# MRIRC/MRI-super-resolution

Measured on AMD Instinct MI355X. Metric: voxels/sec per INR fit (128^3, x4 upscale): train coordinate-steps/s, higher is better.
Workload: dtype f32 as 3 x f16 MFMA products (hi/lo split operands, f32 accumulate); 1 GPU; synthetic 128^3 volume, LR 64x64x128 (N=524288 coords) -> x4 grid 256x256x128; Siren(256,512,3,1) + 128 Fourier features, Adam 1e-4, full-batch MSE; per_gpu_rows=524288, parallelism=1 independent fits (one volume per GPU)

## Files before the change

### mri-super-resolution_amd/csrc/gemm_hp.hip

```cpp
#include "internal.h"
#include "split_fp16.h"

namespace inr {

#include "gemm_hp.inc"
#include "gemm_hp_nt.inc"
#include "gemm_hp_row.inc"
#include "gemm_hp_fwd.inc"

int hp_build_flags() {
    int f = 0;
    if (HP_ABLATE != 0) f |= 2;
    if (HP_A_AUX != 2 || HP_MUL_AUX != 0 || HP_RC_A_AUX != 0 || HP_RC_B_AUX != 0 || HP_HEAD_NT != 0 || HP_UNSCALE_LDEXP != 1 || HP_HEAD_PREFETCH != 1 || HP_COLSUM_TRANSPOSED != 1 || HP_DIAG_NO_OMEGA_STASH != 0) f |= 8;
    return f;
}
tune_int g_stamp_class{-1}, g_stamp_nth{0};
static unsigned long long* hp_stamp_target(int kernel_class) {
    if (!g_stamps || kernel_class != g_stamp_class) return nullptr;
    return g_stamp_nth-- == 0 ? g_stamps : nullptr;
}

tune_int g_hp_stagger{0};
tune_int g_hp_persistent{2};
static int hp_num_cus() {
    static int n = 0;
    if (!n) {
        int dev = 0;
        hipDeviceProp_t prop;
        if (hipGetDevice(&dev) == hipSuccess && hipGetDeviceProperties(&prop, dev) == hipSuccess) n = prop.multiProcessorCount;
        if (n <= 0) n = 256;
    }
    return n;
}
tune_int g_hp_grid_cap{0};
static unsigned hp_persistent_grid(long long tiles) {
    long long g = tiles < hp_num_cus() ? tiles : hp_num_cus();
    const int cap = g_hp_grid_cap;
    if (cap > 0 && g > cap) g = cap;
    return (unsigned)g;
}
bool hp_head_ok(int hidden) { return hidden == 128 || hidden == 256 || hidden == 512 || hidden == 1024; }

size_t hp_prep_part_bytes() { return (size_t)8 * HP_PREP_MAXB * 2 * sizeof(unsigned); }
int hp_weight_prep(const float* const* W, const int* out_f, const int* in_f, int layers, char* planes, HpSlots slots,
                   unsigned* part, float* head_bound, const float* head_W, const float* head_b, int hidden, const unsigned* tmax,
                   const unsigned* wtmax, float inv_count, float omega, hipStream_t stream, const float* const* bias,
// ... 89 lines not shown
    }
    return c;
}

static HpParams hp_kc_params(char* c_hl, const char* a_hl, const char* b_hl, int64_t rows, int width, int k, HpScale sa, HpScale sb,
                             HpScale so, int kernel_class) {
    HpParams p{};
    p.A = a_hl; p.B = b_hl; p.C_hl = c_hl;
    p.M = (int)rows; p.N = width; p.K = k;
    p.pitchA = (long long)k * 4; p.pitchB = (long long)k * 4;
    p.a_rows = rows; p.b_rows = width;
    p.sa = sa; p.sb = sb; p.so = so;
    p.k_per_split = k; p.splits = 1; p.stagger = g_hp_stagger;
    p.stamps = hp_stamp_target(kernel_class);
    return p;
}

template <int EPI>
static int hp_launch_kc(HpParams p, const HpKcChoice& c, hipStream_t stream) {
    constexpr bool INLINE_EPI = EPI == HPE_SINE || EPI == HPE_SINE_STASH || EPI == HPE_MUL;
    const bool narrow = c.family == LF_HP_NARROW;
    const int bm = narrow ? NT_BM : HP_BM, bn = narrow ? NT_BN : HP_BN;
    p.tiles_m = (int)((p.a_rows + bm - 1) / bm);
    p.tiles_n = c.family == LF_HP_ROW ? 1 : (p.N + bn - 1) / bn;
    if (narrow) p.fold_bias = c.fold_bias;
    if (int rc = hp_check_grid(p)) return rc;
    const long long tiles = (long long)p.tiles_m * p.tiles_n;
    const dim3 grid((unsigned)tiles), pgrid(hp_persistent_grid(tiles)), block(narrow ? NT_NTH : HP_NTH);
    bool served = false;
    if (c.family == LF_HP_ROW) {
        hipLaunchKernelGGL((gemm_hp_row_kernel<EPI>), pgrid, block, 0, stream, p);
        served = true;
    }
    if constexpr (EPI != HPE_HEAD) {
        if (c.family == LF_HP_PKD && c.kt == 16) {
            hipLaunchKernelGGL((gemm_hp_pkd_kernel<EPI, 16>), pgrid, block, 0, stream, p);
            served = true;
        } else if (c.family == LF_HP_NARROW) {
            if (c.xzy) hipLaunchKernelGGL((gemm_hp_nt_kernel<EPI, true>), grid, block, 0, stream, p);
            else hipLaunchKernelGGL((gemm_hp_nt_kernel<EPI, false>), grid, block, 0, stream, p);
            served = true;
        }
        if constexpr (EPI != HPE_MUL) {
            if (c.family == LF_HP_PKD && c.kt == 8) {
                hipLaunchKernelGGL((gemm_hp_pkd_kernel<EPI, 8>), pgrid, block, 0, stream, p);
                served = true;
            }
        }
    }
    if constexpr (INLINE_EPI) {
        if (c.family == LF_HP_PKC) {
            hipLaunchKernelGGL((gemm_hp_pkc_kernel<EPI>), pgrid, block, 0, stream, p);
            served = true;
        } else if (c.family == LF_HP_TILE) {
            hipLaunchKernelGGL((gemm_hp_kernel<HP_KC, EPI>), grid, block, 0, stream, p);
            served = true;
        }
    }
    INR_REQUIRE(served, INR_E_INVALID, "hp gemm: no kernel of family %d for epilogue %d at K = %d", c.family, EPI, p.K);
    INR_LAUNCH_CHECK();
    count_launch(c.family);
    return 0;
}

int hp_sine_forward(char* act_hl, float* dact, const char* x_hl, const char* W_hl, const float* bias, int64_t n, int in_f,
                    int out_f, float omega, HpScale sa, HpScale sb, int reverse_m, hipStream_t stream, bool z_only, HpScale so) {
// ... 291 lines not shown
```

### mri-super-resolution_amd/csrc/gemm_hp.inc

```
__device__ __forceinline__ int hp_f(int r) {
    const int p = (r >> 1) & 7;
    return (p & 1) ^ (((p >> 1) & 1) * 5) ^ (((p >> 2) & 1) * 7);
}
__device__ __forceinline__ int hp_f2(int r) { return (r & 3) | (((r >> 3) & 1) << 2); }

#ifndef HP_A_AUX
#define HP_A_AUX 2
#endif
#ifndef HP_HEAD_NT
#define HP_HEAD_NT 0
#endif
#ifndef HP_RC_A_AUX
#define HP_RC_A_AUX 0
#endif
#ifndef HP_RC_B_AUX
#define HP_RC_B_AUX 0
#endif
#ifndef HP_MUL_AUX
#define HP_MUL_AUX 0
#endif
#ifndef HP_COLSUM_TRANSPOSED
#define HP_COLSUM_TRANSPOSED 1
#endif
#ifndef HP_HEAD_PREFETCH
#define HP_HEAD_PREFETCH 1
#endif
#ifndef HP_UNSCALE_LDEXP
#define HP_UNSCALE_LDEXP 1
#endif
#ifndef HP_DIAG_NO_OMEGA_STASH
#define HP_DIAG_NO_OMEGA_STASH 0
#endif
#ifndef HP_ABLATE
#define HP_ABLATE 0
#endif
enum HpMode { HP_KC = 0, HP_RC = 1 };
enum HpEpi { HPE_SINE = 0, HPE_SINE_STASH = 1, HPE_MUL = 2, HPE_SLAB = 3, HPE_Z = 4, HPE_HEAD = 5 };

__device__ __forceinline__ int hp_scale_exp(const HpScale& s) {
    if (s.mul == 0.f) return 0;
    float b = s.mul;
    if (s.meas) b *= __uint_as_float(*s.meas);
    if (s.wn) b *= *s.wn;
    if (!s.wn) return h3_scale_exp(__float_as_uint(b));
    return h3_scale_exp(__float_as_uint(b), s.kmax, -126);
}

__device__ __forceinline__ void hp_atomic_max_bits(unsigned* slot, float v) {
    const unsigned b = __float_as_uint(v);
    if (b > __hip_atomic_load(slot, __ATOMIC_RELAXED, __HIP_MEMORY_SCOPE_AGENT)) atomicMax(slot, b);
}

struct HpParams {
    const char* A;
    const char* B;
    int M, N, K;
    long long pitchA, pitchB;
    long long a_rows, b_rows;
    HpScale sa, sb, so;
    char* C_hl;
    float* C2;
    const float* bias;
    const float* mul;
    float* colsum;
    unsigned* amax_out;
    float omega;
    int tiles_m, tiles_n, splits;
    int k_per_split;
// ... 37 lines not shown
template <int ROWB>
__device__ __forceinline__ half8 hp_tr_read2(const char* lds) {
    typedef unsigned int u32x2 __attribute__((ext_vector_type(2)));
    u32x2 a, b;
    const unsigned addr = (unsigned)(unsigned long long)(__attribute__((address_space(3))) const char*)lds;
    asm volatile("ds_read_b64_tr_b16 %0, %1" : "=v"(a) : "v"(addr));
    asm volatile("ds_read_b64_tr_b16 %0, %1 offset:%2" : "=v"(b) : "v"(addr), "n"(4 * ROWB));
    return __builtin_bit_cast(half8, u32x4{a[0], a[1], b[0], b[1]});
}


__device__ __forceinline__ f32x4 hp_mul_sum(const f32x4& a, const f32x4& b, f32x4& cs) {
#pragma clang fp contract(off)
    const f32x4 o = a * b;
    cs = cs + o;
    return o;
}

__device__ __forceinline__ void hp_split8(const float (&v)[8], float s, u32x4& hi, u32x4& lo) {
    half2v h[4], l[4];
#pragma unroll
    for (int e = 0; e < 4; ++e) h3_split2<true>(v[2 * e], v[2 * e + 1], s, h[e], l[e]);
    hi = __builtin_bit_cast(u32x4, h);
    lo = __builtin_bit_cast(u32x4, l);
}
__device__ __forceinline__ void hp_split8_unit(const float (&v)[8], u32x4& hi, u32x4& lo) {
    half2v h[4], l[4];
#pragma unroll
    for (int e = 0; e < 4; ++e) h3_split2<false>(v[2 * e], v[2 * e + 1], 1.f, h[e], l[e]);
    hi = __builtin_bit_cast(u32x4, h);
    lo = __builtin_bit_cast(u32x4, l);
}

template <int MODE, int EPI>
__device__ __forceinline__ void gemm_hp_body(const HpParams& p, const int block_x) {
    constexpr int EPI_BYTES = 8 * 64 * SUB16 * 4;
    constexpr int SMEM_BYTES = HP_NSTAGE * HP_STAGE > EPI_BYTES ? HP_NSTAGE * HP_STAGE : EPI_BYTES;
    __shared__ __attribute__((aligned(1024))) char smem[SMEM_BYTES];
    constexpr bool KC = MODE == HP_KC;
    constexpr int A_ROWB = KC ? 128 : 512, B_ROWB = KC ? 128 : 1024;

    const int tid = threadIdx.x;
    const int lane = tid & 63, wave = __builtin_amdgcn_readfirstlane(tid >> 6);
    const int wm = wave >> 2, wn = wave & 3;
    const int g = lane >> 4, l16 = lane & 15;

    const int total = p.tiles_m * p.tiles_n * p.splits;
    int logical = xcd_remap(block_x, total);
    int tile_n = logical % p.tiles_n;
    logical /= p.tiles_n;
    int tile_m = logical % p.tiles_m;
    int split = logical / p.tiles_m;
    if (p.reverse_m) {
        if (p.splits > 1) split = p.splits - 1 - split;
        else tile_m = p.tiles_m - 1 - tile_m;
    }
    const int m0 = tile_m * HP_BM, n0 = tile_n * HP_BN;
    const int k_begin = split * p.k_per_split;
    const int k_end = min(p.K, k_begin + p.k_per_split);
    const int ktiles = (k_end - k_begin + HP_BK - 1) / HP_BK;

    __amdgpu_buffer_rsrc_t srdA, srdB;
    int step_a, step_b;
    if (KC) {
        srdA = hp_srd(p.A + (long long)m0 * p.pitchA, (p.a_rows - m0) * p.pitchA);
        srdB = hp_srd(p.B + (long long)n0 * p.pitchB, (p.b_rows - n0) * p.pitchB);
        step_a = step_b = 128;
    } else {
        const long long ra = min((long long)(k_end - k_begin), p.a_rows - k_begin);
        srdA = hp_srd(p.A + (long long)k_begin * p.pitchA + (m0 >> 5) * 128, ra * p.pitchA - (m0 >> 5) * 128);
        srdB = hp_srd(p.B + (long long)k_begin * p.pitchB + (n0 >> 5) * 128, ra * p.pitchB - (n0 >> 5) * 128);
        step_a = (int)(32 * p.pitchA);
        step_b = (int)(32 * p.pitchB);
    }
    int vdma[6];
#pragma unroll
    for (int i = 0; i < 6; ++i) {
        const int q = wave + 8 * i;
        if (KC) {
            const int row = 8 * (i < 2 ? q : q - 16) + (lane >> 3);
            const int c = (lane & 7) ^ hp_f(row);
            vdma[i] = row * (int)(i < 2 ? p.pitchA : p.pitchB) + c * 16;
        } else if (i < 2) {
            const int row = 2 * q + (lane >> 5), u = lane & 31;
            const int ch = (u >> 1) ^ hp_f2(row);
            vdma[i] = row * (int)p.pitchA + ch * 32 + (u & 1) * 16;
        } else {
            const int row = q - 16, u = lane;
            const int ch = (u >> 1) ^ hp_f2(row);
            vdma[i] = row * (int)p.pitchB + ch * 32 + (u & 1) * 16;
        }
    }
    int soff_a = KC ? (k_begin >> 5) * 128 : 0, soff_b = soff_a;
    auto dma_part = [&](int stage, int part) {
        char* S = smem + stage * HP_STAGE;
#pragma unroll
        for (int i = 0; i < 6; ++i) {
            if ((i >> 1) != part) continue;
            const int q = wave + 8 * i;
            if (!KC && i < 2)
                __builtin_amdgcn_raw_ptr_buffer_load_lds(srdA, (__attribute__((address_space(3))) void*)(S + q * 1024), 16, vdma[i],
                                                         soff_a, 0, HP_RC_A_AUX);
            else if (!KC)
                __builtin_amdgcn_raw_ptr_buffer_load_lds(srdB, (__attribute__((address_space(3))) void*)(S + q * 1024), 16, vdma[i],
                                                         soff_b, 0, HP_RC_B_AUX);
            else
                __builtin_amdgcn_raw_ptr_buffer_load_lds(i < 2 ? srdA : srdB, (__attribute__((address_space(3))) void*)(S + q * 1024),
                                                         16, vdma[i], i < 2 ? soff_a : soff_b, 0, 0);
        }
        if (part == 2) {
            soff_a += step_a;
            soff_b += step_b;
        }
    };
    auto dma = [&](int stage) {
        dma_part(stage, 0);
        dma_part(stage, 1);
        dma_part(stage, 2);
    };

    int fa[KC ? 2 : 8], fb[KC ? 2 : 8];
    if (KC) {
        const int fx = (g ^ hp_f(l16)) << 4;
        fa[0] = (64 * wm + l16) * 128 + fx;
        fa[1] = fa[0] ^ 64;
        fb[0] = HP_A_IMG + (64 * wn + l16) * 128 + fx;
        fb[1] = fb[0] ^ 64;
    } else {
        const int q = l16 >> 2, p4 = l16 & 3, row = 8 * g + q, f2 = hp_f2(row);
#pragma unroll
        for (int t = 0; t < 4; ++t)
#pragma unroll
            for (int lo = 0; lo < 2; ++lo) {
                const int mi = 4 * wm + t, ca = 4 * (mi >> 1) + (mi & 1) + 2 * lo;
                fa[2 * t + lo] = row * 512 + (ca ^ f2) * 32 + p4 * 8;
                const int ni = 4 * wn + t, cb = 4 * (ni >> 1) + (ni & 1) + 2 * lo;
                fb[2 * t + lo] = HP_A_IMG + row * 1024 + (cb ^ f2) * 32 + p4 * 8;
            }
    }
    auto frag_a = [&](const char* S, int i, int lo) -> half8 {
        if (KC) return *reinterpret_cast<const half8*>(S + fa[lo] + i * 2048);
        return hp_tr_read2<512>(S + fa[2 * i + lo]);
    };
    auto frag_b = [&](const char* S, int i, int lo) -> half8 {
        if (KC) return *reinterpret_cast<const half8*>(S + fb[lo] + i * 2048);
        return hp_tr_read2<1024>(S + fb[2 * i + lo]);
// ... 6 lines not shown
        for (int j = 0; j < 4; ++j) acc[i][j] = f32x4v{0.f, 0.f, 0.f, 0.f};
    half8 ah[2][4], bh[2][4], al[4], bl[4];

    HP_STAMP(0);
    if (ktiles > 0) dma(0);
    if (ktiles > 1) dma(1);
    if (ktiles > 2) dma(2);
    if (ktiles > 2) __builtin_amdgcn_s_waitcnt(0x0F70 | 12);
    else if (ktiles > 1) __builtin_amdgcn_s_waitcnt(0x0F70 | 6);
    else __builtin_amdgcn_s_waitcnt(0x0F70);
    __builtin_amdgcn_s_barrier();
    if (ktiles > 0) {
#pragma unroll
        for (int i = 0; i < 4; ++i) {
            ah[0][i] = frag_a(smem, i, 0);
            bl[i] = frag_b(smem, i, 1);
            al[i] = frag_a(smem, i, 1);
            bh[0][i] = frag_b(smem, i, 0);
        }
    }
    HP_STAMP(1);

    constexpr int NRD = KC ? 8 : 16;
    auto body = [&](auto par_c, auto st_c, int t) {
        constexpr int PAR = decltype(par_c)::value, ST = decltype(st_c)::value;
        const char* S1 = smem + ((ST + 1) % 3) * HP_STAGE;
        const bool more3 = t + 3 < ktiles;
        if (t == 7) HP_STAMP(5);
        if (t + 2 < ktiles) __builtin_amdgcn_s_waitcnt(0x0070 | 6);
        else __builtin_amdgcn_s_waitcnt(0x0070);
        __builtin_amdgcn_s_barrier();
        __builtin_amdgcn_sched_barrier(0);
        if (t == 7) HP_STAMP(6);
        if (more3) dma_part(ST, 0);
        h3_mfma16(acc, ah[PAR], bl);
        __builtin_amdgcn_sched_barrier(0);
        if (t == 7) HP_STAMP(7);
        if (more3) dma_part(ST, 1);
        if (KC) {
#pragma unroll
            for (int i = 0; i < 4; ++i) {
                bl[i] = frag_b(S1, i, 1);
                ah[PAR ^ 1][i] = frag_a(S1, i, 0);
            }
            h3_mfma16(acc, al, bh[PAR]);
            h3_sched<16, 0, 0, NRD, 0, 0>();
        } else {
#pragma unroll
            for (int i = 0; i < 4; ++i)
#pragma unroll
                for (int j = 0; j < 4; ++j) {
                    acc[i][j] = __builtin_amdgcn_mfma_f32_16x16x32_f16(al[i], bh[PAR][j], acc[i][j], 0, 0, 0);
                    if (j == 1) bl[i] = frag_b(S1, i, 1);
                    if (j == 3) ah[PAR ^ 1][i] = frag_a(S1, i, 0);
                }
        }
        __builtin_amdgcn_sched_barrier(0);
        if (t == 7) HP_STAMP(8);
        if (more3) dma_part(ST, 2);
        if (KC) {
#pragma unroll
            for (int i = 0; i < 4; ++i) {
                al[i] = frag_a(S1, i, 1);
                bh[PAR ^ 1][i] = frag_b(S1, i, 0);
            }
            h3_mfma16(acc, ah[PAR], bh[PAR]);
            h3_sched<16, 0, 0, NRD, 0, 0>();
        } else {
#pragma unroll
            for (int i = 0; i < 4; ++i)
#pragma unroll
                for (int j = 0; j < 4; ++j) {
                    acc[i][j] = __builtin_amdgcn_mfma_f32_16x16x32_f16(ah[PAR][i], bh[PAR][j], acc[i][j], 0, 0, 0);
                    if (j == 1) al[i] = frag_a(S1, i, 1);
                    if (j == 3) bh[PAR ^ 1][i] = frag_b(S1, i, 0);
                }
        }
        __builtin_amdgcn_sched_barrier(0);
        if (t == 7) HP_STAMP(9);
    };
    {
        using I0 = std::integral_constant<int, 0>;
        using I1 = std::integral_constant<int, 1>;
        using I2 = std::integral_constant<int, 2>;
        int t = 0;
        for (; t + 6 <= ktiles; t += 6) {
            body(I0{}, I0{}, t);
            body(I1{}, I1{}, t + 1);
            body(I0{}, I2{}, t + 2);
            body(I1{}, I0{}, t + 3);
            body(I0{}, I1{}, t + 4);
            body(I1{}, I2{}, t + 5);
        }
        if (t < ktiles) {
            body(I0{}, I0{}, t);
            if (t + 1 < ktiles) {
                body(I1{}, I1{}, t + 1);
                if (t + 2 < ktiles) {
                    body(I0{}, I2{}, t + 2);
                    if (t + 3 < ktiles) {
// ... 848 lines not shown
    while (true) {
        int t = 0;
        for (; t + 1 < ktiles; t += 2) {
            body(P0{}, t);
            body(P1{}, t + 1);
        }
        if (t < ktiles) {
            body(P0{}, t);
#pragma unroll
            for (int i = 0; i < 4; ++i) {
                ah[0][i] = ah[1][i];
                bh[0][i] = bh[1][i];
            }
        }
        HP_STAMP(2);
        if (!(HP_ABLATE & 4)) epilogue();
        else if (acc[0][0][0] == 12345.678f) p.C_hl[0] = (char)acc[1][1][1];
        HP_STAMP(4);
        if (!has_next) break;
        if (nxt.n0 != cur.n0) load_bias(nxt.n0);
        zero_acc();
        pend = 1;
        cur = nxt;
        vp += G;
        has_next = vp + G < total;
        if (has_next) nxt = decode(vp + G);
    }
    if (EPI == HPE_MUL && p.amax_out) {
        omax_run = wave_max(omax_run);
        if (lane == 0) hp_atomic_max_bits(p.amax_out, omax_run);
    }
}

template <int I, int N, typename F>
__device__ __forceinline__ void hp_static_for(F&& f) {
    if constexpr (I < N) {
        f(std::integral_constant<int, I>{});
        hp_static_for<I + 1, N>(f);
    }
}

template <int EPI, int KT>
__global__ void __launch_bounds__(HP_NTH, 2) gemm_hp_pkd_kernel(const HpParams p) {
    __shared__ __attribute__((aligned(1024))) char smem[HP_NSTAGE * HP_STAGE + 8 * HP_EPI_WAVE];
    constexpr int STORES = EPI == HPE_SINE_STASH ? 4 : 2;
    static_assert(EPI != HPE_SLAB, "row-split slabs are the one-block-per-tile kernel's business");
    constexpr int MULS = EPI == HPE_MUL ? 2 : 0;

    const int tid = threadIdx.x;
    const int lane = tid & 63, wave = __builtin_amdgcn_readfirstlane(tid >> 6);
    const int wm = wave >> 2, wn = wave & 3;
    const int g = lane >> 4, l16 = lane & 15;
    const int total = p.tiles_m * p.tiles_n;
    const int G = gridDim.x;

    struct Tile {
        int m0, n0;
        __amdgpu_buffer_rsrc_t srdA, srdB;
    };
    auto decode = [&](int vp) {
        int logical = xcd_remap(vp, total);
        Tile t;
        const int tn = logical % p.tiles_n, tm = logical / p.tiles_n;
        t.m0 = (p.reverse_m ? p.tiles_m - 1 - tm : tm) * HP_BM;
        t.n0 = tn * HP_BN;
        t.srdA = hp_srd(p.A + (long long)t.m0 * p.pitchA, (p.a_rows - t.m0) * p.pitchA);
        t.srdB = hp_srd(p.B + (long long)t.n0 * p.pitchB, (p.b_rows - t.n0) * p.pitchB);
        return t;
    };
    int vp = blockIdx.x;
    Tile cur = decode(vp), nxt = cur;
    bool has_next = vp + G < total;
    if (has_next) nxt = decode(vp + G);
    int prv_m0 = 0, prv_n0 = 0;
    bool have_prev = false;

    const int drow = 8 * wave + (lane >> 3);
    const int dslot = ((lane & 7) ^ hp_f(drow)) * 16;
    const int vdmaA = drow * (int)p.pitchA + dslot, vdmaB = drow * (int)p.pitchB + dslot;
    const int pieceA = 64 * (int)p.pitchA, pieceB = 64 * (int)p.pitchB;
    auto dma_part = [&](int stage_off, int j, int part) {
        char* S = smem + stage_off;
        const bool from_next = j >= KT;
        const int soff = (from_next ? j - KT : j) * 128;
        const __amdgpu_buffer_rsrc_t sa = from_next ? nxt.srdA : cur.srdA, sb = from_next ? nxt.srdB : cur.srdB;
#pragma unroll
        for (int i = 0; i < 6; ++i) {
            if ((i >> 1) != part) continue;
            const int q = wave + 8 * i;
            if (i < 2)
                __builtin_amdgcn_raw_ptr_buffer_load_lds(sa, (__attribute__((address_space(3))) void*)(S + q * 1024), 16, vdmaA,
                                                         soff + i * pieceA, 0, HP_A_AUX);
            else
                __builtin_amdgcn_raw_ptr_buffer_load_lds(sb, (__attribute__((address_space(3))) void*)(S + q * 1024), 16, vdmaB,
                                                         soff + (i - 2) * pieceB, 0, 0);
        }
    };

    const int fx = (g ^ hp_f(l16)) << 4;
    const int fa_hi = (64 * wm + l16) * 128 + fx, fa_lo = fa_hi ^ 64;
    const int fb_hi = HP_A_IMG + (64 * wn + l16) * 128 + fx, fb_lo = fb_hi ^ 64;

    const int ka = hp_scale_exp(p.sa), kb = hp_scale_exp(p.sb);
    float bias_s[4] = {0.f, 0.f, 0.f, 0.f};
    auto load_bias = [&](int n0) {
        if (EPI == HPE_MUL || !p.bias) return;
        const float upa = h3_pow2(ka), upb = h3_pow2(kb);
#pragma unroll
        for (int j = 0; j < 4; ++j) {
            const int col = n0 + 64 * wn + 16 * j + l16;
            const float b = p.bias[col < p.N ? col : p.N - 1];
            bias_s[j] = col < p.N ? (b * upa) * upb : 0.f;
        }
    };
    load_bias(cur.n0);
    f32x4v acc[4][4], accP[4][4];
    half8 ah[4], al[4], bh[4], bl[4];
    auto init_acc = [&]() {
#pragma unroll
        for (int i = 0; i < 4; ++i)
#pragma unroll
            for (int j = 0; j < 4; ++j) acc[i][j] = f32x4v{bias_s[j], bias_s[j], bias_s[j], bias_s[j]};
    };
    init_acc();

    const int er = lane >> 2, ec = (lane & 3) * 8;
    float* const stg = reinterpret_cast<float*>(smem + HP_NSTAGE * HP_STAGE + wave * HP_EPI_WAVE);
    const float inv_a = h3_pow2(-ka), inv_b = h3_pow2(-kb);
    const float so = h3_pow2(hp_scale_exp(p.so));
    f32x4 mul0 = {0.f, 0.f, 0.f, 0.f}, mul1 = mul0;
    f32x4 cs0 = {0.f, 0.f, 0.f, 0.f}, cs1 = cs0;
    float omax_run = 0.f;

    auto load_mul = [&](int c, f32x4& d0, f32x4& d1) {
        const __amdgpu_buffer_rsrc_t srdMul =
            hp_srd((const char*)p.mul + (long long)prv_m0 * p.N * 4, (long long)min(p.M - prv_m0, HP_BM) * p.N * 4);
        const int row = 64 * wm + 16 * (c & 3) + er, cc = prv_n0 + 64 * wn + 32 * (c >> 2) + ec;
        const int vo = cc < p.N ? (row * p.N + cc) * 4 : 0x7FFFFF00;
        d0 = __builtin_bit_cast(f32x4, __builtin_amdgcn_raw_buffer_load_b128(srdMul, vo, 0, HP_MUL_AUX));
        d1 = __builtin_bit_cast(f32x4, __builtin_amdgcn_raw_buffer_load_b128(srdMul, vo + 16, 0, HP_MUL_AUX));
    };
    auto chunk_park = [&](auto cc) {
        constexpr int c = decltype(cc)::value, i = c & 3, jp = c >> 2;
#pragma unroll
        for (int jj = 0; jj < 2; ++jj)
#pragma unroll
            for (int r = 0; r < 4; ++r)
                stg[(4 * g + r) * 32 + jj * 16 + l16] =
                    HP_UNSCALE_LDEXP ? __builtin_amdgcn_ldexpf(accP[i][2 * jp + jj][r], -(ka + kb)) : accP[i][2 * jp + jj][r] * inv_a * inv_b;
    };
    f32x4 cv0, cv1;
    auto chunk_read = [&]() {
        __builtin_amdgcn_s_waitcnt(0xC07F);
        __builtin_amdgcn_wave_barrier();
        cv0 = *reinterpret_cast<const f32x4*>(stg + er * 32 + ec);
        cv1 = *reinterpret_cast<const f32x4*>(stg + er * 32 + ec + 4);
    };
    auto chunk_finish = [&](auto cc) {
        constexpr int c = decltype(cc)::value, i = c & 3, jp = c >> 2;
        const long long first = (long long)prv_m0 * p.N * 4;
        const long long win = (long long)min(p.M - prv_m0, HP_BM) * p.N * 4;
        const __amdgpu_buffer_rsrc_t srdHL = hp_srd(p.C_hl + first, win);
        const int row = 64 * wm + 16 * i + er, col = prv_n0 + 64 * wn + 32 * jp + ec;
        const bool ok = col < p.N;
        const int vhl = ok ? row * p.N * 4 + (col >> 5) * 128 + (col & 31) * 2 : 0x7FFFFF00;
        if (EPI == HPE_MUL) {
            const f32x4 o0 = hp_mul_sum(cv0, mul0, cs0), o1 = hp_mul_sum(cv1, mul1, cs1);
            omax_run = fmaxf(omax_run, fmaxf(fmaxf(fmaxf(fabsf(o0[0]), fabsf(o0[1])), fmaxf(fabsf(o0[2]), fabsf(o0[3]))),
                                             fmaxf(fmaxf(fabsf(o1[0]), fabsf(o1[1])), fmaxf(fabsf(o1[2]), fabsf(o1[3])))));
            const float ov[8] = {o0[0], o0[1], o0[2], o0[3], o1[0], o1[1], o1[2], o1[3]};
            u32x4 hi, lo;
            hp_split8(ov, so, hi, lo);
            __builtin_amdgcn_raw_buffer_store_b128(hi, srdHL, vhl, 0, 0);
            __builtin_amdgcn_raw_buffer_store_b128(lo, srdHL, vhl + 64, 0, 0);
            if (i == 3) {
                const long long cbytes = p.colsum ? 2ll * p.tiles_m * p.N * 4 : 0;
                const __amdgpu_buffer_rsrc_t srdCS = hp_srd(p.colsum ? (const void*)p.colsum : (const void*)p.C_hl, cbytes);
                if (HP_COLSUM_TRANSPOSED) {
                    const float total = hp_colsum_fold(cs0, cs1, lane);
                    const int vcs = (lane < 32 && ok) ? (((prv_m0 / HP_BM) * 2 + wm) * p.N + col + hp_colsum_index(lane)) * 4 : 0x7FFFFF00;
                    __builtin_amdgcn_raw_buffer_store_b32(__builtin_bit_cast(unsigned, total), srdCS, vcs, 0, 0);
                } else {
#pragma unroll
                    for (int e = 0; e < 4; ++e) {
                        cs0[e] += __shfl_xor(cs0[e], 4, 64);
                        cs1[e] += __shfl_xor(cs1[e], 4, 64);
                        cs0[e] += __shfl_xor(cs0[e], 8, 64);
                        cs1[e] += __shfl_xor(cs1[e], 8, 64);
                        cs0[e] += __shfl_xor(cs0[e], 16, 64);
                        cs1[e] += __shfl_xor(cs1[e], 16, 64);
                        cs0[e] += __shfl_xor(cs0[e], 32, 64);
                        cs1[e] += __shfl_xor(cs1[e], 32, 64);
                    }
                    const int vcs = (lane < 4 && ok) ? (((prv_m0 / HP_BM) * 2 + wm) * p.N + col) * 4 : 0x7FFFFF00;
                    buf_store4(cs0, srdCS, vcs, 0);
                    buf_store4(cs1, srdCS, vcs + 16, 0);
                }
                cs0 = f32x4{0.f, 0.f, 0.f, 0.f};
                cs1 = cs0;
            }
        } else if (EPI == HPE_Z) {
            const __amdgpu_buffer_rsrc_t srdC2 = hp_srd((const char*)p.C2 + first, win);
            const int v32 = ok ? (row * p.N + col) * 4 : 0x7FFFFF00;
            buf_store4(cv0, srdC2, v32, 0);
            buf_store4(cv1, srdC2, v32 + 16, 0);
        } else {
            const f32x4 z0 = p.omega * cv0, z1 = p.omega * cv1;
            float sv[8], cvv[8];
            {
                f32x2_t s2[4], c2[4];
                sincos_f32x2_fast(f32x2_t{z0[0], z0[1]}, s2[0], c2[0]);
                sincos_f32x2_fast(f32x2_t{z0[2], z0[3]}, s2[1], c2[1]);
                sincos_f32x2_fast(f32x2_t{z1[0], z1[1]}, s2[2], c2[2]);
                sincos_f32x2_fast(f32x2_t{z1[2], z1[3]}, s2[3], c2[3]);
#pragma unroll
                for (int e = 0; e < 8; ++e) {
                    sv[e] = s2[e >> 1][e & 1];
                    cvv[e] = c2[e >> 1][e & 1];
                }
            }
            u32x4 hi, lo;
            hp_split8(sv, so, hi, lo);
            __builtin_amdgcn_raw_buffer_store_b128(hi, srdHL, vhl, 0, 0);
            __builtin_amdgcn_raw_buffer_store_b128(lo, srdHL, vhl + 64, 0, 0);
            if (EPI == HPE_SINE_STASH) {
                const __amdgpu_buffer_rsrc_t srdC2 = hp_srd((const char*)p.C2 + first, win);
                const int v32 = ok ? (row * p.N + col) * 4 : 0x7FFFFF00;
                if (HP_DIAG_NO_OMEGA_STASH) {
                    buf_store4(f32x4{cvv[0], cvv[1], cvv[2], cvv[3]}, srdC2, v32, 0);
                    buf_store4(f32x4{cvv[4], cvv[5], cvv[6], cvv[7]}, srdC2, v32 + 16, 0);
                } else {
                    buf_store4(p.omega * f32x4{cvv[0], cvv[1], cvv[2], cvv[3]}, srdC2, v32, 0);
                    buf_store4(p.omega * f32x4{cvv[4], cvv[5], cvv[6], cvv[7]}, srdC2, v32 + 16, 0);
                }
            }
        }
    };
    auto epilogue_now = [&]() {
        hp_static_for<0, 8>([&](auto cc) {
            constexpr int c = decltype(cc)::value;
            chunk_park(cc);
            if (EPI == HPE_MUL) load_mul(c, mul0, mul1);
            chunk_read();
            chunk_finish(cc);
            __builtin_amdgcn_s_waitcnt(0xC07F);
            __builtin_amdgcn_wave_barrier();
        });
    };

    if (p.stagger > 0) {
        for (int k = ((blockIdx.x >> 3) + blockIdx.x) & 7; k > 0; --k)
            for (int q = 0; q < p.stagger; q += 100) __builtin_amdgcn_s_sleep(100);
    }
    HP_STAMP(0);
    int so3[3] = {0, HP_STAGE, 2 * HP_STAGE};
#pragma unroll
    for (int part = 0; part < 3; ++part) dma_part(so3[0], 0, part);
#pragma unroll
    for (int part = 0; part < 3; ++part) dma_part(so3[1], 1, part);
    dma_part(so3[2], 2, 0);
    dma_part(so3[2], 2, 1);
    __builtin_amdgcn_s_waitcnt(hp_vmcnt(10));
    __builtin_amdgcn_s_barrier();
#pragma unroll
    for (int i = 0; i < 4; ++i) {
        ah[i] = *reinterpret_cast<const half8*>(smem + so3[0] + fa_hi + i * 2048);
        bl[i] = *reinterpret_cast<const half8*>(smem + so3[0] + fb_lo + i * 2048);
    }
    HP_STAMP(1);
    int last_extra = 0;

    constexpr int PERIOD = KT / 8;
    static_assert(KT % 8 == 0 && KT >= 8, "one chunk per KT / 8 iterations");
    auto iteration = [&](auto tc) {
        constexpr int t = decltype(tc)::value;
        constexpr bool SLOT = t % PERIOD == 0;
        constexpr int c = t / PERIOD;
        const bool mine = SLOT && have_prev && !(HP_ABLATE & 4);
        const char* S = smem + so3[t % 3];
        const char* S1 = smem + so3[(t + 1) % 3];
        const bool more2 = t + 2 < KT || has_next, more3 = t + 3 < KT || has_next;
        if (EPI == HPE_MUL && mine) load_mul(c, mul0, mul1);
        if (more2 && !(HP_ABLATE & 1)) dma_part(so3[(t + 2) % 3], t + 2, 2);
        if (!(HP_ABLATE & 8)) {
#pragma unroll
            for (int i = 0; i < 4; ++i) {
                al[i] = *reinterpret_cast<const half8*>(S + fa_lo + i * 2048);
                bh[i] = *reinterpret_cast<const half8*>(S + fb_hi + i * 2048);
            }
        }
        if (!(HP_ABLATE & 2)) h3_mfma16(acc, ah, bl);
        h3_sched<16, 0, 0, 8, 0, 0>();
        __builtin_amdgcn_sched_barrier(0);
        {
            const bool now = mine && MULS > 0;
            if (!more2) __builtin_amdgcn_s_waitcnt(hp_vmcnt(0) & 0xF0FF);
            else if (last_extra && now) __builtin_amdgcn_s_waitcnt(hp_vmcnt(6 + STORES + MULS) & 0xF0FF);
            else if (last_extra) __builtin_amdgcn_s_waitcnt(hp_vmcnt(6 + STORES) & 0xF0FF);
            else if (now) __builtin_amdgcn_s_waitcnt(hp_vmcnt(6 + MULS) & 0xF0FF);
            else __builtin_amdgcn_s_waitcnt(hp_vmcnt(6) & 0xF0FF);
        }
        __builtin_amdgcn_s_barrier();
        __builtin_amdgcn_sched_barrier(0);
        if (more3 && !(HP_ABLATE & 1)) dma_part(so3[t % 3], t + 3, 0);
        if (mine) chunk_park(std::integral_constant<int, c>{});
        if (!(HP_ABLATE & 8)) {
#pragma unroll
            for (int i = 0; i < 4; ++i) bl[i] = *reinterpret_cast<const half8*>(S1 + fb_lo + i * 2048);
        }
        if (!(HP_ABLATE & 2)) h3_mfma16(acc, ah, bh);
        __builtin_amdgcn_sched_barrier(0);
        if (more3 && !(HP_ABLATE & 1)) dma_part(so3[t % 3], t + 3, 1);
        if (mine) chunk_read();
        if (!(HP_ABLATE & 8)) {
#pragma unroll
            for (int i = 0; i < 4; ++i) ah[i] = *reinterpret_cast<const half8*>(S1 + fa_hi + i * 2048);
        }
        if (!(HP_ABLATE & 2)) h3_mfma16(acc, al, bh);
        if (mine) chunk_finish(std::integral_constant<int, c>{});
        __builtin_amdgcn_sched_barrier(0);
        last_extra = mine ? 1 : 0;
    };
    while (true) {
        hp_static_for<0, KT>(iteration);
        HP_STAMP(2);
        have_prev = true;
#pragma unroll
        for (int i = 0; i < 4; ++i)
#pragma unroll
            for (int j = 0; j < 4; ++j) accP[i][j] = acc[i][j];
        prv_m0 = cur.m0;
        prv_n0 = cur.n0;
        if (!has_next) break;
        last_extra = 0;
        if (nxt.n0 != cur.n0) load_bias(nxt.n0);
        init_acc();
        {
            const int a = so3[KT % 3], b = so3[(KT + 1) % 3], c2 = so3[(KT + 2) % 3];
            so3[0] = a;
            so3[1] = b;
            so3[2] = c2;
        }
        cur = nxt;
        vp += G;
        has_next = vp + G < total;
        if (has_next) nxt = decode(vp + G);
    }
    if (!(HP_ABLATE & 4)) epilogue_now();
    else if (accP[0][0][0] == 12345.678f) p.C_hl[0] = (char)accP[1][1][1];
    HP_STAMP(4);
    if (EPI == HPE_MUL && p.amax_out) {
        omax_run = wave_max(omax_run);
        if (lane == 0) hp_atomic_max_bits(p.amax_out, omax_run);
    }
}
```

### mri-super-resolution_amd/csrc/split_fp16.h

```cpp
#pragma once
#include "common.h"

namespace inr {

typedef _Float16 half8 __attribute__((ext_vector_type(8)));
typedef _Float16 half4v __attribute__((ext_vector_type(4)));
typedef _Float16 half2v __attribute__((ext_vector_type(2)));
typedef float f32x4v __attribute__((ext_vector_type(4)));

constexpr int SUB16 = 68;

__device__ __forceinline__ int xcd_remap(int pid, int total) {
    const int q = total >> 3, r = total & 7;
    const int xcd = pid & 7, idx = pid >> 3;
    const int base = (xcd < r) ? xcd * (q + 1) : r * (q + 1) + (xcd - r) * q;
    return base + idx;
}

__device__ __forceinline__ f32x4 buf_load4(__amdgpu_buffer_rsrc_t srd, int voff, int soff) {
    const u32x4 v = __builtin_amdgcn_raw_buffer_load_b128(srd, voff, soff, 0);
    return __builtin_bit_cast(f32x4, v);
}
__device__ __forceinline__ void buf_store4(f32x4 v, __amdgpu_buffer_rsrc_t srd, int voff, int row_off) {
    __builtin_amdgcn_raw_buffer_store_b128(__builtin_bit_cast(u32x4, v), srd, voff + row_off, 0, 0);
// ... 21 lines not shown
    if (SCALED) {
        hi = h3_cvt_rn(v0 * s, v1 * s);
        const float r0 = __builtin_fmaf(v0, s, -(float)hi[0]), r1 = __builtin_fmaf(v1, s, -(float)hi[1]);
        lo = h3_cvt_rn(r0, r1);
    } else {
        hi = h3_cvt_rn(v0, v1);
        const float r0 = v0 - (float)hi[0], r1 = v1 - (float)hi[1];
        lo = h3_cvt_rn(r0, r1);
    }
}

template <int NM, int NV, int NW, int NR, int NG, int I>
__device__ __forceinline__ void h3_sched() {
    if constexpr (I < NM) {
        __builtin_amdgcn_sched_group_barrier(0x008, 1, 0);
        constexpr int v = (I + 1) * NV / NM - I * NV / NM;
        if constexpr (v > 0) __builtin_amdgcn_sched_group_barrier(0x002, v, 0);
        constexpr int w = (I + 1) * NW / NM - I * NW / NM;
        if constexpr (w > 0) __builtin_amdgcn_sched_group_barrier(0x200, w, 0);
        constexpr int r = (I + 1) * NR / NM - I * NR / NM;
        if constexpr (r > 0) __builtin_amdgcn_sched_group_barrier(0x100, r, 0);
        constexpr int g = (I + 1) * NG / NM - I * NG / NM;
        if constexpr (g > 0) __builtin_amdgcn_sched_group_barrier(0x020, g, 0);
        h3_sched<NM, NV, NW, NR, NG, I + 1>();
    }
}

__device__ __forceinline__ void h3_mfma16(f32x4v (&acc)[4][4], const half8 (&a)[4], const half8 (&b)[4]) {
#pragma unroll
    for (int i = 0; i < 4; ++i)
#pragma unroll
        for (int j = 0; j < 4; ++j) acc[i][j] = __builtin_amdgcn_mfma_f32_16x16x32_f16(a[i], b[j], acc[i][j], 0, 0, 0);
}

}
```

Baseline: 63.23 million voxels/s.

## Interleave DMA refills into MFMA tails, prefetch mul operand, hoist per-tile SRDs

In the deferred-epilogue (pkd) GEMM kernel, the global-to-LDS DMA refill pieces are moved from the start of each MFMA phase to after the fragment reads, with sched_group_barriers placing them between specific MFMAs. The HPE_MUL epilogue's multiplier loads are issued one step ahead, and buffer resource descriptors for C_hl, C2, mul and colsum are built once per tile instead of in every chunk. The goal is to hide VMEM issue latency behind MFMA work and cut scalar descriptor setup. A new host check requires pitch to equal 4*K for this kernel, since the DMA now uses a compile-time pitch. The RC-mode tail variant exists but is off by default (bit 2 is not set).

```diff
diff --git a/mri-super-resolution_amd/csrc/gemm_hp.hip b/mri-super-resolution_amd/csrc/gemm_hp.hip
--- a/mri-super-resolution_amd/csrc/gemm_hp.hip
+++ b/mri-super-resolution_amd/csrc/gemm_hp.hip
@@ -11,7 +11,7 @@
 int hp_build_flags() {
     int f = 0;
     if (HP_ABLATE != 0) f |= 2;
-    if (HP_A_AUX != 2 || HP_MUL_AUX != 0 || HP_RC_A_AUX != 0 || HP_RC_B_AUX != 0 || HP_HEAD_NT != 0 || HP_UNSCALE_LDEXP != 1 || HP_HEAD_PREFETCH != 1 || HP_COLSUM_TRANSPOSED != 1 || HP_DIAG_NO_OMEGA_STASH != 0) f |= 8;
+    if (HP_A_AUX != 2 || HP_MUL_AUX != 0 || HP_RC_A_AUX != 0 || HP_RC_B_AUX != 0 || HP_HEAD_NT != 0 || HP_UNSCALE_LDEXP != 1 || HP_HEAD_PREFETCH != 1 || HP_COLSUM_TRANSPOSED != 1 || HP_DIAG_NO_OMEGA_STASH != 0 || HP_REFILL_TAIL != 1 || HP_MUL_AHEAD != 1 || HP_TILE_SRD != 1) f |= 8;
     return f;
 }
 tune_int g_stamp_class{-1}, g_stamp_nth{0};
@@ -167,6 +167,8 @@
         hipLaunchKernelGGL((gemm_hp_row_kernel<EPI>), pgrid, block, 0, stream, p);
         served = true;
     }
+    if (c.family == LF_HP_PKD)
+        INR_REQUIRE(p.K == c.kt * HP_BK && p.pitchA == 4ll * p.K && p.pitchB == 4ll * p.K, INR_E_INVALID, "hp gemm: deferred-epilogue kernel at pitch %lld / %lld, K = %d", p.pitchA, p.pitchB, p.K);
     if constexpr (EPI != HPE_HEAD) {
         if (c.family == LF_HP_PKD && c.kt == 16) {
             hipLaunchKernelGGL((gemm_hp_pkd_kernel<EPI, 16>), pgrid, block, 0, stream, p);
diff --git a/mri-super-resolution_amd/csrc/gemm_hp.inc b/mri-super-resolution_amd/csrc/gemm_hp.inc
--- a/mri-super-resolution_amd/csrc/gemm_hp.inc
+++ b/mri-super-resolution_amd/csrc/gemm_hp.inc
@@ -34,6 +34,15 @@
 #ifndef HP_ABLATE
 #define HP_ABLATE 0
 #endif
+#ifndef HP_REFILL_TAIL
+#define HP_REFILL_TAIL 1
+#endif
+#ifndef HP_MUL_AHEAD
+#define HP_MUL_AHEAD 1
+#endif
+#ifndef HP_TILE_SRD
+#define HP_TILE_SRD 1
+#endif
 enum HpMode { HP_KC = 0, HP_RC = 1 };
 enum HpEpi { HPE_SINE = 0, HPE_SINE_STASH = 1, HPE_MUL = 2, HPE_SLAB = 3, HPE_Z = 4, HPE_HEAD = 5 };
 
@@ -137,6 +146,14 @@
     lo = __builtin_bit_cast(u32x4, l);
 }
 
+template <int I, int N, typename F>
+__device__ __forceinline__ void hp_static_for(F&& f) {
+    if constexpr (I < N) {
+        f(std::integral_constant<int, I>{});
+        hp_static_for<I + 1, N>(f);
+    }
+}
+
 template <int MODE, int EPI>
 __device__ __forceinline__ void gemm_hp_body(const HpParams& p, const int block_x) {
     constexpr int EPI_BYTES = 8 * 64 * SUB16 * 4;
@@ -197,26 +214,27 @@
         }
     }
     int soff_a = KC ? (k_begin >> 5) * 128 : 0, soff_b = soff_a;
+    auto dma_piece = [&](int stage, int i) {
+        char* S = smem + stage * HP_STAGE;
+        const int q = wave + 8 * i;
+        if (!KC && i < 2)
+            __builtin_amdgcn_raw_ptr_buffer_load_lds(srdA, (__attribute__((address_space(3))) void*)(S + q * 1024), 16, vdma[i], soff_a, 0,
+                                                     HP_RC_A_AUX);
+        else if (!KC)
+            __builtin_amdgcn_raw_ptr_buffer_load_lds(srdB, (__attribute__((address_space(3))) void*)(S + q * 1024), 16, vdma[i], soff_b, 0,
+                                                     HP_RC_B_AUX);
+        else
+            __builtin_amdgcn_raw_ptr_buffer_load_lds(i < 2 ? srdA : srdB, (__attribute__((address_space(3))) void*)(S + q * 1024), 16,
+                                                     vdma[i], i < 2 ? soff_a : soff_b, 0, 0);
+    };
+    auto dma_advance = [&]() {
+        soff_a += step_a;
+        soff_b += step_b;
+    };
     auto dma_part = [&](int stage, int part) {
-        char* S = smem + stage * HP_STAGE;
-#pragma unroll
-        for (int i = 0; i < 6; ++i) {
-            if ((i >> 1) != part) continue;
-            const int q = wave + 8 * i;
-            if (!KC && i < 2)
-                __builtin_amdgcn_raw_ptr_buffer_load_lds(srdA, (__attribute__((address_space(3))) void*)(S + q * 1024), 16, vdma[i],
-                                                         soff_a, 0, HP_RC_A_AUX);
-            else if (!KC)
-                __builtin_amdgcn_raw_ptr_buffer_load_lds(srdB, (__attribute__((address_space(3))) void*)(S + q * 1024), 16, vdma[i],
-                                                         soff_b, 0, HP_RC_B_AUX);
-            else
-                __builtin_amdgcn_raw_ptr_buffer_load_lds(i < 2 ? srdA : srdB, (__attribute__((address_space(3))) void*)(S + q * 1024),
-                                                         16, vdma[i], i < 2 ? soff_a : soff_b, 0, 0);
-        }
-        if (part == 2) {
-            soff_a += step_a;
-            soff_b += step_b;
-        }
+        dma_piece(stage, 2 * part);
+        dma_piece(stage, 2 * part + 1);
+        if (part == 2) dma_advance();
     };
     auto dma = [&](int stage) {
         dma_part(stage, 0);
@@ -289,11 +307,27 @@
         __builtin_amdgcn_s_barrier();
         __builtin_amdgcn_sched_barrier(0);
         if (t == 7) HP_STAMP(6);
-        if (more3) dma_part(ST, 0);
-        h3_mfma16(acc, ah[PAR], bl);
+        constexpr bool TAIL = !KC && (HP_REFILL_TAIL & 2) != 0;
+        auto tail_pieces = [&](auto q_c, int part) {
+            constexpr int q = decltype(q_c)::value;
+            if (q != 9 && q != 12) return;
+            __builtin_amdgcn_sched_barrier(0);
+            if (more3) dma_piece(ST, 2 * part + (q == 12));
+            if (more3 && q == 12 && part == 2) dma_advance();
+        };
+        if (TAIL) {
+            hp_static_for<0, 16>([&](auto q_c) {
+                constexpr int q = decltype(q_c)::value, i = q >> 2, j = q & 3;
+                acc[i][j] = __builtin_amdgcn_mfma_f32_16x16x32_f16(ah[PAR][i], bl[j], acc[i][j], 0, 0, 0);
+                tail_pieces(q_c, 0);
+            });
+        } else {
+            if (more3) dma_part(ST, 0);
+            h3_mfma16(acc, ah[PAR], bl);
+        }
         __builtin_amdgcn_sched_barrier(0);
         if (t == 7) HP_STAMP(7);
-        if (more3) dma_part(ST, 1);
+        if (!TAIL && more3) dma_part(ST, 1);
         if (KC) {
 #pragma unroll
             for (int i = 0; i < 4; ++i) {
@@ -302,6 +336,14 @@
             }
             h3_mfma16(acc, al, bh[PAR]);
             h3_sched<16, 0, 0, NRD, 0, 0>();
+        } else if (TAIL) {
+            hp_static_for<0, 16>([&](auto q_c) {
+                constexpr int q = decltype(q_c)::value, i = q >> 2, j = q & 3;
+                acc[i][j] = __builtin_amdgcn_mfma_f32_16x16x32_f16(al[i], bh[PAR][j], acc[i][j], 0, 0, 0);
+                if constexpr (q < 8 && (q & 1) == 0) bl[q >> 1] = frag_b(S1, q >> 1, 1);
+                if constexpr (q < 8 && (q & 1) == 1) ah[PAR ^ 1][q >> 1] = frag_a(S1, q >> 1, 0);
+                tail_pieces(q_c, 1);
+            });
         } else {
 #pragma unroll
             for (int i = 0; i < 4; ++i)
@@ -314,7 +356,7 @@
         }
         __builtin_amdgcn_sched_barrier(0);
         if (t == 7) HP_STAMP(8);
-        if (more3) dma_part(ST, 2);
+        if (!TAIL && more3) dma_part(ST, 2);
         if (KC) {
 #pragma unroll
             for (int i = 0; i < 4; ++i) {
@@ -323,6 +365,14 @@
             }
             h3_mfma16(acc, ah[PAR], bh[PAR]);
             h3_sched<16, 0, 0, NRD, 0, 0>();
+        } else if (TAIL) {
+            hp_static_for<0, 16>([&](auto q_c) {
+                constexpr int q = decltype(q_c)::value, i = q >> 2, j = q & 3;
+                acc[i][j] = __builtin_amdgcn_mfma_f32_16x16x32_f16(ah[PAR][i], bh[PAR][j], acc[i][j], 0, 0, 0);
+                if constexpr (q < 8 && (q & 1) == 0) al[q >> 1] = frag_a(S1, q >> 1, 1);
+                if constexpr (q < 8 && (q & 1) == 1) bh[PAR ^ 1][q >> 1] = frag_b(S1, q >> 1, 0);
+                tail_pieces(q_c, 2);
+            });
         } else {
 #pragma unroll
             for (int i = 0; i < 4; ++i)
@@ -1237,11 +1287,17 @@
     }
 }
 
-template <int I, int N, typename F>
-__device__ __forceinline__ void hp_static_for(F&& f) {
-    if constexpr (I < N) {
-        f(std::integral_constant<int, I>{});
-        hp_static_for<I + 1, N>(f);
+#ifndef HP_REFILL_RD
+#define HP_REFILL_RD 10
+#endif
+template <int NR, int I>
+__device__ __forceinline__ void hp_sched_refill() {
+    if constexpr (I < 16) {
+        __builtin_amdgcn_sched_group_barrier(0x008, 1, 0);
+        constexpr int r = I < HP_REFILL_RD ? (I + 1) * NR / HP_REFILL_RD - I * NR / HP_REFILL_RD : 0;
+        if constexpr (r > 0) __builtin_amdgcn_sched_group_barrier(0x100, r, 0);
+        if constexpr (I == 9 || I == 12) __builtin_amdgcn_sched_group_barrier(0x020, 1, 0);
+        hp_sched_refill<NR, I + 1>();
     }
 }
 
@@ -1282,24 +1338,26 @@
 
     const int drow = 8 * wave + (lane >> 3);
     const int dslot = ((lane & 7) ^ hp_f(drow)) * 16;
-    const int vdmaA = drow * (int)p.pitchA + dslot, vdmaB = drow * (int)p.pitchB + dslot;
-    const int pieceA = 64 * (int)p.pitchA, pieceB = 64 * (int)p.pitchB;
-    auto dma_part = [&](int stage_off, int j, int part) {
+    constexpr int PITCH = KT * 128;
+    const int pitchA = HP_TILE_SRD ? PITCH : (int)p.pitchA, pitchB = HP_TILE_SRD ? PITCH : (int)p.pitchB;
+    const int vdmaA = drow * pitchA + dslot, vdmaB = drow * pitchB + dslot;
+    const int pieceA = 64 * pitchA, pieceB = 64 * pitchB;
+    auto dma_piece = [&](int stage_off, int j, int i) {
         char* S = smem + stage_off;
         const bool from_next = j >= KT;
         const int soff = (from_next ? j - KT : j) * 128;
         const __amdgpu_buffer_rsrc_t sa = from_next ? nxt.srdA : cur.srdA, sb = from_next ? nxt.srdB : cur.srdB;
-#pragma unroll
-        for (int i = 0; i < 6; ++i) {
-            if ((i >> 1) != part) continue;
-            const int q = wave + 8 * i;
-            if (i < 2)
-                __builtin_amdgcn_raw_ptr_buffer_load_lds(sa, (__attribute__((address_space(3))) void*)(S + q * 1024), 16, vdmaA,
-                                                         soff + i * pieceA, 0, HP_A_AUX);
-            else
-                __builtin_amdgcn_raw_ptr_buffer_load_lds(sb, (__attribute__((address_space(3))) void*)(S + q * 1024), 16, vdmaB,
-                                                         soff + (i - 2) * pieceB, 0, 0);
-        }
+        const int q = wave + 8 * i;
+        if (i < 2)
+            __builtin_amdgcn_raw_ptr_buffer_load_lds(sa, (__attribute__((address_space(3))) void*)(S + q * 1024), 16, vdmaA, soff + i * pieceA, 0,
+                                                     HP_A_AUX);
+        else
+            __builtin_amdgcn_raw_ptr_buffer_load_lds(sb, (__attribute__((address_space(3))) void*)(S + q * 1024), 16, vdmaB,
+                                                     soff + (i - 2) * pieceB, 0, 0);
+    };
+    auto dma_part = [&](int stage_off, int j, int part) {
+        dma_piece(stage_off, j, 2 * part);
+        dma_piece(stage_off, j, 2 * part + 1);
     };
 
     const int fx = (g ^ hp_f(l16)) << 4;
@@ -1337,10 +1395,22 @@
     f32x4 cs0 = {0.f, 0.f, 0.f, 0.f}, cs1 = cs0;
     float omax_run = 0.f;
 
+    auto win_of = [&](int m0) { return (long long)min(p.M - m0, HP_BM) * p.N * 4; };
+    auto mk_hl = [&](int m0) { return hp_srd(p.C_hl + (long long)m0 * p.N * 4, win_of(m0)); };
+    auto mk_c2 = [&](int m0) { return hp_srd((const char*)p.C2 + (long long)m0 * p.N * 4, win_of(m0)); };
+    auto mk_mul = [&](int m0) { return hp_srd((const char*)p.mul + (long long)m0 * p.N * 4, win_of(m0)); };
+    auto mk_cs = [&]() { return hp_srd(p.colsum ? (const void*)p.colsum : (const void*)p.C_hl, p.colsum ? 2ll * p.tiles_m * p.N * 4 : 0); };
+    __amdgpu_buffer_rsrc_t srdHL_t = hp_srd(p.C_hl, 0), srdC2_t = srdHL_t, srdMul_t = srdHL_t;
+    const __amdgpu_buffer_rsrc_t srdCS_t = mk_cs();
+    int mul_m0 = 0, mul_n0 = 0;
+    auto set_mul_tile = [&](int m0, int n0) {
+        mul_m0 = m0;
+        mul_n0 = n0;
+        if (HP_TILE_SRD && EPI == HPE_MUL) srdMul_t = mk_mul(m0);
+    };
     auto load_mul = [&](int c, f32x4& d0, f32x4& d1) {
-        const __amdgpu_buffer_rsrc_t srdMul =
-            hp_srd((const char*)p.mul + (long long)prv_m0 * p.N * 4, (long long)min(p.M - prv_m0, HP_BM) * p.N * 4);
-        const int row = 64 * wm + 16 * (c & 3) + er, cc = prv_n0 + 64 * wn + 32 * (c >> 2) + ec;
+        const __amdgpu_buffer_rsrc_t srdMul = HP_TILE_SRD ? srdMul_t : mk_mul(mul_m0);
+        const int row = 64 * wm + 16 * (c & 3) + er, cc = mul_n0 + 64 * wn + 32 * (c >> 2) + ec;
         const int vo = cc < p.N ? (row * p.N + cc) * 4 : 0x7FFFFF00;
         d0 = __builtin_bit_cast(f32x4, __builtin_amdgcn_raw_buffer_load_b128(srdMul, vo, 0, HP_MUL_AUX));
         d1 = __builtin_bit_cast(f32x4, __builtin_amdgcn_raw_buffer_load_b128(srdMul, vo + 16, 0, HP_MUL_AUX));
@@ -1363,9 +1433,7 @@
     };
     auto chunk_finish = [&](auto cc) {
         constexpr int c = decltype(cc)::value, i = c & 3, jp = c >> 2;
-        const long long first = (long long)prv_m0 * p.N * 4;
-        const long long win = (long long)min(p.M - prv_m0, HP_BM) * p.N * 4;
-        const __amdgpu_buffer_rsrc_t srdHL = hp_srd(p.C_hl + first, win);
+        const __amdgpu_buffer_rsrc_t srdHL = HP_TILE_SRD ? srdHL_t : mk_hl(prv_m0);
         const int row = 64 * wm + 16 * i + er, col = prv_n0 + 64 * wn + 32 * jp + ec;
         const bool ok = col < p.N;
         const int vhl = ok ? row * p.N * 4 + (col >> 5) * 128 + (col & 31) * 2 : 0x7FFFFF00;
@@ -1379,8 +1447,7 @@
             __builtin_amdgcn_raw_buffer_store_b128(hi, srdHL, vhl, 0, 0);
             __builtin_amdgcn_raw_buffer_store_b128(lo, srdHL, vhl + 64, 0, 0);
             if (i == 3) {
-                const long long cbytes = p.colsum ? 2ll * p.tiles_m * p.N * 4 : 0;
-                const __amdgpu_buffer_rsrc_t srdCS = hp_srd(p.colsum ? (const void*)p.colsum : (const void*)p.C_hl, cbytes);
+                const __amdgpu_buffer_rsrc_t srdCS = HP_TILE_SRD ? srdCS_t : mk_cs();
                 if (HP_COLSUM_TRANSPOSED) {
                     const float total = hp_colsum_fold(cs0, cs1, lane);
                     const int vcs = (lane < 32 && ok) ? (((prv_m0 / HP_BM) * 2 + wm) * p.N + col + hp_colsum_index(lane)) * 4 : 0x7FFFFF00;
@@ -1405,7 +1472,7 @@
                 cs1 = cs0;
             }
         } else if (EPI == HPE_Z) {
-            const __amdgpu_buffer_rsrc_t srdC2 = hp_srd((const char*)p.C2 + first, win);
+            const __amdgpu_buffer_rsrc_t srdC2 = HP_TILE_SRD ? srdC2_t : mk_c2(prv_m0);
             const int v32 = ok ? (row * p.N + col) * 4 : 0x7FFFFF00;
             buf_store4(cv0, srdC2, v32, 0);
             buf_store4(cv1, srdC2, v32 + 16, 0);
@@ -1429,7 +1496,7 @@
             __builtin_amdgcn_raw_buffer_store_b128(hi, srdHL, vhl, 0, 0);
             __builtin_amdgcn_raw_buffer_store_b128(lo, srdHL, vhl + 64, 0, 0);
             if (EPI == HPE_SINE_STASH) {
-                const __amdgpu_buffer_rsrc_t srdC2 = hp_srd((const char*)p.C2 + first, win);
+                const __amdgpu_buffer_rsrc_t srdC2 = HP_TILE_SRD ? srdC2_t : mk_c2(prv_m0);
                 const int v32 = ok ? (row * p.N + col) * 4 : 0x7FFFFF00;
                 if (HP_DIAG_NO_OMEGA_STASH) {
                     buf_store4(f32x4{cvv[0], cvv[1], cvv[2], cvv[3]}, srdC2, v32, 0);
@@ -1445,7 +1512,7 @@
         hp_static_for<0, 8>([&](auto cc) {
             constexpr int c = decltype(cc)::value;
             chunk_park(cc);
-            if (EPI == HPE_MUL) load_mul(c, mul0, mul1);
+            if (EPI == HPE_MUL && !(HP_MUL_AHEAD && KT == 16 && c == 0)) load_mul(c, mul0, mul1);
             chunk_read();
             chunk_finish(cc);
             __builtin_amdgcn_s_waitcnt(0xC07F);
@@ -1485,8 +1552,23 @@
         const char* S = smem + so3[t % 3];
         const char* S1 = smem + so3[(t + 1) % 3];
         const bool more2 = t + 2 < KT || has_next, more3 = t + 3 < KT || has_next;
-        if (EPI == HPE_MUL && mine) load_mul(c, mul0, mul1);
-        if (more2 && !(HP_ABLATE & 1)) dma_part(so3[(t + 2) % 3], t + 2, 2);
+        constexpr bool AHEAD = HP_MUL_AHEAD && EPI == HPE_MUL && PERIOD == 2;
+        constexpr int ld_c = AHEAD ? ((t + 1) / 2) % 8 : c;
+        bool ld_now = EPI == HPE_MUL && mine;
+        if constexpr (AHEAD) {
+            if constexpr (t == KT - 1) {
+                set_mul_tile(cur.m0, cur.n0);
+                ld_now = !(HP_ABLATE & 4);
+            } else {
+                ld_now = t % 2 == 1 && have_prev && !(HP_ABLATE & 4);
+            }
+        }
+        constexpr bool TAIL = (HP_REFILL_TAIL & (EPI == HPE_MUL ? 4 : 1)) != 0;
+        constexpr int SB = t == 6 ? 5 : t == 7 ? 10 : -1;
+        if constexpr (SB > 0) HP_STAMP(SB);
+        if (ld_now) load_mul(ld_c, mul0, mul1);
+        __builtin_amdgcn_sched_barrier(0);
+        if (!TAIL && more2 && !(HP_ABLATE & 1)) dma_part(so3[(t + 2) % 3], t + 2, 2);
         if (!(HP_ABLATE & 8)) {
 #pragma unroll
             for (int i = 0; i < 4; ++i) {
@@ -1494,11 +1576,14 @@
                 bh[i] = *reinterpret_cast<const half8*>(S + fb_hi + i * 2048);
             }
         }
+        if (TAIL && more2 && !(HP_ABLATE & 1)) dma_part(so3[(t + 2) % 3], t + 2, 2);
         if (!(HP_ABLATE & 2)) h3_mfma16(acc, ah, bl);
-        h3_sched<16, 0, 0, 8, 0, 0>();
+        if (TAIL) hp_sched_refill<8, 0>();
+        else h3_sched<16, 0, 0, 8, 0, 0>();
         __builtin_amdgcn_sched_barrier(0);
+        if constexpr (SB > 0) HP_STAMP(SB + 1);
         {
-            const bool now = mine && MULS > 0;
+            const bool now = ld_now && MULS > 0;
             if (!more2) __builtin_amdgcn_s_waitcnt(hp_vmcnt(0) & 0xF0FF);
             else if (last_extra && now) __builtin_amdgcn_s_waitcnt(hp_vmcnt(6 + STORES + MULS) & 0xF0FF);
             else if (last_extra) __builtin_amdgcn_s_waitcnt(hp_vmcnt(6 + STORES) & 0xF0FF);
@@ -1507,23 +1592,30 @@
         }
         __builtin_amdgcn_s_barrier();
         __builtin_amdgcn_sched_barrier(0);
-        if (more3 && !(HP_ABLATE & 1)) dma_part(so3[t % 3], t + 3, 0);
+        if constexpr (SB > 0) HP_STAMP(SB + 2);
+        if (!TAIL && more3 && !(HP_ABLATE & 1)) dma_part(so3[t % 3], t + 3, 0);
         if (mine) chunk_park(std::integral_constant<int, c>{});
         if (!(HP_ABLATE & 8)) {
 #pragma unroll
             for (int i = 0; i < 4; ++i) bl[i] = *reinterpret_cast<const half8*>(S1 + fb_lo + i * 2048);
         }
+        if (TAIL && more3 && !(HP_ABLATE & 1)) dma_part(so3[t % 3], t + 3, 0);
         if (!(HP_ABLATE & 2)) h3_mfma16(acc, ah, bh);
+        if (TAIL && !(HP_ABLATE & 10)) hp_sched_refill<4, 0>();
         __builtin_amdgcn_sched_barrier(0);
-        if (more3 && !(HP_ABLATE & 1)) dma_part(so3[t % 3], t + 3, 1);
+        if constexpr (SB > 0) HP_STAMP(SB + 3);
+        if (!TAIL && more3 && !(HP_ABLATE & 1)) dma_part(so3[t % 3], t + 3, 1);
         if (mine) chunk_read();
         if (!(HP_ABLATE & 8)) {
 #pragma unroll
             for (int i = 0; i < 4; ++i) ah[i] = *reinterpret_cast<const half8*>(S1 + fa_hi + i * 2048);
         }
+        if (TAIL && more3 && !(HP_ABLATE & 1)) dma_part(so3[t % 3], t + 3, 1);
         if (!(HP_ABLATE & 2)) h3_mfma16(acc, al, bh);
+        if (TAIL && !(HP_ABLATE & 10)) hp_sched_refill<4, 0>();
         if (mine) chunk_finish(std::integral_constant<int, c>{});
         __builtin_amdgcn_sched_barrier(0);
+        if constexpr (SB > 0) HP_STAMP(SB + 4);
         last_extra = mine ? 1 : 0;
     };
     while (true) {
@@ -1536,6 +1628,11 @@
             for (int j = 0; j < 4; ++j) accP[i][j] = acc[i][j];
         prv_m0 = cur.m0;
         prv_n0 = cur.n0;
+        if (HP_TILE_SRD) {
+            srdHL_t = mk_hl(prv_m0);
+            if (EPI == HPE_SINE_STASH || EPI == HPE_Z) srdC2_t = mk_c2(prv_m0);
+        }
+        if (!(HP_MUL_AHEAD && EPI == HPE_MUL && KT == 16)) set_mul_tile(prv_m0, prv_n0);
         if (!has_next) break;
         last_extra = 0;
         if (nxt.n0 != cur.n0) load_bias(nxt.n0);
diff --git a/mri-super-resolution_amd/csrc/split_fp16.h b/mri-super-resolution_amd/csrc/split_fp16.h
--- a/mri-super-resolution_amd/csrc/split_fp16.h
+++ b/mri-super-resolution_amd/csrc/split_fp16.h
@@ -77,5 +77,10 @@
 #pragma unroll
         for (int j = 0; j < 4; ++j) acc[i][j] = __builtin_amdgcn_mfma_f32_16x16x32_f16(a[i], b[j], acc[i][j], 0, 0, 0);
 }
+template <int LO, int HI>
+__device__ __forceinline__ void h3_mfma16_part(f32x4v (&acc)[4][4], const half8 (&a)[4], const half8 (&b)[4]) {
+#pragma unroll
+    for (int q = LO; q < HI; ++q) acc[q >> 2][q & 3] = __builtin_amdgcn_mfma_f32_16x16x32_f16(a[q >> 2], b[q & 3], acc[q >> 2][q & 3], 0, 0, 0);
+}
 
 }
```

Result: slower. 62.39 million voxels/s (-1.3%).
